# gavrissh/training-operator

Hardware: AMD Instinct MI355X
Metric: job×node fit evals/sec + gang placements/sec, 1M-node inventory, 1/2/4/8 GPUs (higher is better)
Workload: dtype int64

## Files before the change

training-operator_amd/csrc/pe_engine.cpp:

```cpp
#include <hip/hip_runtime.h>
#include <rccl/rccl.h>

#include <immintrin.h>
#include <pthread.h>
#include <sched.h>

#include <algorithm>
#include <deque>
#include <condition_variable>
#include <atomic>
#include <chrono>
#include <exception>
#include <functional>
#include <thread>
#include <cstdio>
#include <cstdlib>
#include <cstring>
#include <memory>
#include <mutex>
#include <new>
#include <numeric>
#include <string>
#include <unordered_map>
#include <vector>
// ... 353 lines not shown
  DevBuf<uint64_t> dm_table;
  HostBuf<uint64_t> dm_hslots;
  HostBuf<uint32_t> dm_hnodes;
  HostBuf<pe::DomPick> dm_hpicks;
  DevBuf<pe::DomPick> dm_picks;
  DevBuf<pe::DomSel> dm_sel;
  HostBuf<pe::DomSel> dm_hsel;
  std::vector<pe::DomPick> dm_upicks;
  std::vector<int32_t> dm_ptab, dm_pof;
  DevBuf<ReqRec> g_groups;
  DevBuf<uint64_t> g_cand, g_bound;
  DevBuf<int32_t> g_cnt;
  DevBuf<uint8_t> g_out, g_gath;
  DevBuf<int64_t> g_upd;
  DevBuf<uint64_t> g_kn;
  DevBuf<uint32_t> g_lo;
  HostBuf<ReqRec> h_groups, h_groups2;
  HostBuf<ReqRec> h_groupsx[2];
  HostBuf<uint8_t> h_outx[2];
  HostBuf<int64_t> h_updx[2];
  uint32_t walk_gen = 0;
  int pin_cpu = -2;
  HostBuf<uint8_t> h_out, h_out2, h_own;
  HostBuf<uint8_t> h_merged;
  HostBuf<uint8_t> h_xg[4];
  std::vector<const uint64_t*> x_lists;
  std::vector<int32_t> x_ns, x_hd;
  HostBuf<int64_t> h_upd;
  bool walk = true;
  int64_t resort_nodes = 20480;
  int64_t w_est = 0;
  struct WalkSet {
    DevBuf<uint64_t> sk, rmin;
    DevBuf<int64_t> sr, rmax;
    DevBuf<uint32_t> sl, pos, ror, inovl, ovidx, ovlab;
    DevBuf<int64_t> ovres;
    DevBuf<uint64_t> ovkn;
    DevBuf<int32_t> ovl, ovln;
    void release() {
      sk.release(); rmin.release(); sr.release(); rmax.release(); sl.release(); pos.release(); ror.release();
      inovl.release(); ovidx.release(); ovlab.release(); ovres.release(); ovkn.release(); ovl.release(); ovln.release();
    }
  } ws[2];
  int w_cur = 0;
  bool w_pending = false;
  int64_t w_pend_est = 0;
  int64_t w_pend_windows = 0;
  hipStream_t w_s2 = nullptr;
  hipEvent_t w_ev_snap = nullptr, w_ev_done = nullptr;
  DevBuf<uint64_t> w_kin;
  DevBuf<uint32_t> w_slow;
  DevBuf<uint8_t> w_temp;
  DevBuf<uint32_t> w_flush;
  DevBuf<unsigned long long> w_stat;
  DevBuf<uint64_t> g_xstatus;
  pe_stats stats{};

  ~pe_ctx() {
    (void)hipSetDevice(device);
    if (comm_abort.joinable()) comm_abort.join();
    if (stream) (void)hipStreamSynchronize(stream);
    res0.release(); res.release(); labels.release(); island.release(); n_upd.release();
    fit_jobs.release(); fit_jobs32.release(); res32.release(); mask.release();
    code_vals.release(); code_needs.release(); code_jobs.release(); code_x.release(); counts.release(); h_counts.release();
    planes.release(); plane_jobs.release();
    lds_spec_d.release(); lds_vals.release(); lds_codes.release(); lds_ranks.release(); lds_aux.release(); lds_slots.release(); lds_rows.release();
    a_stage.release(); a_outh.release(); a_segoff.release(); a_flag.release(); a_ctr.release();
    for (hipEvent_t e : a_ev) (void)hipEventDestroy(e);
    if (a_h2d) (void)hipStreamSynchronize(a_h2d);
    for (hipEvent_t e : a_ev_h2d) (void)hipEventDestroy(e);
    if (a_h2d) (void)hipStreamDestroy(a_h2d);
    a_dstage.release();
    a_jgo.release(); a_mm.release(); a_rep.release(); a_gco.release(); a_mem.release();
    a_req.release(); a_out.release(); a_fl.release(); a_pres.release(); a_ovf.release();
    aw_stage.release(); aw_outh.release(); aw_dev.release();
    cp_hshapes.release(); cp_hout.release(); cp_shapes.release(); cp_part.release(); cp_out.release();
    dm_table.release(); dm_hslots.release(); dm_hnodes.release(); dm_hpicks.release();
    dm_picks.release(); dm_sel.release(); dm_hsel.release();
    for (hipEvent_t e : cp_ev)
      if (e) (void)hipEventDestroy(e);
    g_groups.release(); g_cand.release(); g_bound.release(); g_cnt.release(); g_out.release(); g_gath.release();
    g_upd.release(); g_kn.release(); g_lo.release(); h_groups.release(); h_groups2.release(); h_out.release(); h_out2.release(); h_own.release(); h_merged.release(); h_upd.release();
    for (auto& x : h_xg) x.release();
    for (int i = 0; i < 2; ++i) {
      h_groupsx[i].release();
      h_outx[i].release();
      h_updx[i].release();
    }
    if (w_s2) (void)hipStreamSynchronize(w_s2);
    for (auto& x : ws) x.release();
    w_kin.release(); w_slow.release(); w_temp.release(); w_stat.release(); w_flush.release(); g_xstatus.release();
    if (w_ev_snap) (void)hipEventDestroy(w_ev_snap);
    if (w_ev_done) (void)hipEventDestroy(w_ev_done);
    if (w_s2) (void)hipStreamDestroy(w_s2);
    if (comm) (void)ncclCommDestroy(comm);
    if (stream) (void)hipStreamDestroy(stream);
  }
};

namespace {

void rccl_abort(pe_ctx* ctx) {
  if (!ctx->comm) return;
  ncclComm_t c = ctx->comm;
  ctx->comm = nullptr;
  ctx->comm_aborted = true;
  const int dev = ctx->device;
  ctx->comm_abort = std::thread([c, dev] {
    (void)hipSetDevice(dev);
    (void)ncclCommAbort(c);
  });
}

template <class F>
int guarded(pe_ctx* ctx, F&& body) {
  if (!ctx) return PE_EINVAL;
  std::lock_guard<std::mutex> lk(ctx->mu);
  ctx->err.clear();
  try {
    hipchk(hipSetDevice(ctx->device), "hipSetDevice");
    return body();
  } catch (const PeError& e) {
    ctx->err = e.msg;
    return e.code;
  } catch (const std::bad_alloc&) {
    ctx->err = "host allocation failed";
    return PE_ENOMEM;
  } catch (const pe::CollectiveTimeout& e) {
    ctx->err = e.what();
    rccl_abort(ctx);
    return PE_ERCCL;
  } catch (const pe::ExchangeError& e) {
    ctx->err = e.what();
    return PE_ERCCL;
  } catch (const std::runtime_error& e) {
    ctx->err = e.what();
    return PE_EHIP;
  } catch (...) {
    ctx->err = "unexpected C++ exception";
    return PE_EINVAL;
  }
}

void need_ptr(const void* p, const char* name) {
// ... 2388 lines not shown
      std::vector<double>& d; std::vector<double>& e; std::vector<double>& f;
      ~TraceOut() {
        if (!on || a.empty()) return;
        auto pr = [](const char* n, std::vector<double>& v) {
          if (v.empty()) return;
          std::sort(v.begin(), v.end());
          double sum = 0;
          for (double x : v) sum += x;
          std::fprintf(stderr, "%s n %zu sum %.2f ms mean %.1f us p10 %.1f p50 %.1f p90 %.1f max %.1f\n", n, v.size(),
                       sum / 1e3, sum / v.size(), v[v.size() / 10], v[v.size() / 2], v[v.size() * 9 / 10], v.back());
        };
        pr("wait   ", a);
        pr("resolve", b);
        pr("post   ", c);
        pr("xspin  ", d);
        pr("xmerge ", e);
        pr("xblock ", f);
        auto sib = [](int cpu) {
          char path[128], buf[64] = {0};
          std::snprintf(path, sizeof path, "/sys/devices/system/cpu/cpu%d/topology/thread_siblings_list", cpu);
          FILE* f = std::fopen(path, "r");
          if (f) {
            if (!std::fgets(buf, sizeof buf, f)) buf[0] = 0;
            std::fclose(f);
          }
          buf[std::strcspn(buf, "\n")] = 0;
          return std::string(buf);
        };
        const int mc = sched_getcpu();
        std::fprintf(stderr, "cpus: main %d (siblings %s) helper %d (siblings %s)\n", mc, sib(mc).c_str(), helper_cpu,
                     helper_cpu >= 0 ? sib(helper_cpu).c_str() : "-");
      }
    } trace_out{helper_cpu, trace, tr_wait, tr_res, tr_post, tr_xspin, tr_xmerge, tr_xblock};
    int64_t dump_left = std::getenv("PE_DUMP_MAX_WINDOWS") ? std::atoll(std::getenv("PE_DUMP_MAX_WINDOWS")) : INT64_MAX;
    const size_t gb = pe::cand_group_bytes(K);
    const int Wmax = ctx->window_groups;
    const int Wpad = (int)round_up(Wmax, pe::SC_GT);
    const int nwaves = (int)std::max<int64_t>(1, (ctx->Ns + pe::SC_SPAN - 1) / pe::SC_SPAN);
    hipchk(ctx->g_groups.ensure(Wpad), "alloc groups");
    hipchk(ctx->h_groups.ensure(Wpad, kZeroCopy), "alloc pinned groups");
    hipchk(ctx->g_cand.ensure((size_t)Wpad * nwaves * 64), "alloc cand");
    hipchk(ctx->g_cnt.ensure((size_t)Wpad * nwaves), "alloc cnt");
    hipchk(ctx->g_bound.ensure((size_t)Wpad * nwaves), "alloc bound");
    hipchk(ctx->g_out.ensure((size_t)Wmax * gb), "alloc out");
    hipchk(ctx->h_out.ensure((size_t)Wmax * gb * ctx->world, kZeroCopy), "alloc pinned out");
    if (ctx->pipeline) hipchk(ctx->h_out2.ensure((size_t)Wmax * gb * ctx->world, kZeroCopy), "alloc pinned out");
    if (ctx->world > 1 || ctx->comm) {
      hipchk(ctx->g_gath.ensure((size_t)Wmax * gb * ctx->world), "alloc gather");
      hipchk(ctx->h_own.ensure((size_t)Wmax * gb, kZeroCopy), "alloc pinned own");
    }
    const bool wev = walk && std::getenv("PE_WALK_EVENTS") != nullptr;
    const bool wflush = walk && std::getenv("PE_WALK_FLUSH") != nullptr;
    if (wflush) hipchk(ctx->w_flush.ensure((size_t)512 << 20), "alloc flush buffer");
    std::vector<std::pair<hipEvent_t, hipEvent_t>> walk_events;
    struct EventsFree {
      std::vector<std::pair<hipEvent_t, hipEvent_t>>& v;
      ~EventsFree() {
        for (auto& p : v) {
          (void)hipEventDestroy(p.first);
          (void)hipEventDestroy(p.second);
        }
      }
    } events_free{walk_events};
    int64_t walk_launch_groups = 0;
    std::vector<pe::GroupCands> cands;
    hipStream_t s = ctx->stream;
    const bool use_exchange = ctx->exchange && !(ctx->world == 1 && !ctx->comm);
    const bool pipelined = ctx->pipeline;
    int cb = 0;
    std::unique_ptr<SpinWorker> worker;
    struct Pin {
      cpu_set_t old_set, l3;
      bool on = false;
      Pin(int rank, int world, int& picked) {
        if (std::getenv("PE_NO_PIN") || pthread_getaffinity_np(pthread_self(), sizeof(old_set), &old_set) != 0)
          return;
        if (world > 1 && picked == -2) picked = pe::l3_pick(old_set, rank);
        const int cpu = world > 1 ? picked : sched_getcpu();
        if (!pe::l3_cpus(cpu, &l3)) return;
        CPU_AND(&l3, &l3, &old_set);
        on = CPU_COUNT(&l3) >= 3 && pthread_setaffinity_np(pthread_self(), sizeof(l3), &l3) == 0;
      }
      ~Pin() {
        if (on) (void)pthread_setaffinity_np(pthread_self(), sizeof(old_set), &old_set);
      }
    } pin(ctx->rank, ctx->world, ctx->pin_cpu);
    if (pipelined) {
      worker.reset(new SpinWorker(ctx->device));
      if (pin.on) worker->pin(pin.l3);
    }
    if (pin.on) R.pin_helper(pin.l3);
    auto outbuf = [&](int b) { return b == 0 ? ctx->h_out.p : b == 1 ? ctx->h_out2.p : ctx->h_outx[b - 2].p; };
    auto outbufdev = [&](int b) { return b == 0 ? ctx->h_out.dev : b == 1 ? ctx->h_out2.dev : ctx->h_outx[b - 2].dev; };
    const bool direct_out = ctx->world == 1 && !ctx->comm;
    const bool dev_merge = !direct_out && (int64_t)ctx->world * K <= pe::MG_CAP &&
                           ctx->world <= pe::MG_THREADS / 64 && !std::getenv("PE_HOST_MERGE");
    const bool ranked = (std::getenv("PE_MERGE_RANKED") || (ctx->world <= 2 && !std::getenv("PE_MERGE_SORT"))) &&
                        ctx->world <= pe::RM_MAX_WORLD && pe::merge_ranked_lds(ctx->world, K) <= pe::RM_MAX_LDS;
    auto* const merge_fn = ranked ? &pe::launch_merge_ranked : &pe::launch_merge_shards;
    const bool signalled = pipelined && !std::getenv("PE_NO_GROUP_SIGNAL") && (direct_out ? walk : dev_merge);
    bool zc = false;
    pe_host_exchange* const hx = pe::hx_is(ctx->exchange) ? static_cast<pe_host_exchange*>(ctx->exchange_user) : nullptr;
    if (hx && use_exchange && pipelined && signalled && ctx->walk && !std::getenv("PE_NO_ZC_EXCHANGE")) {
      if (ctx->zc_hx != hx) {
        const uint8_t ok = ctx->world <= pe::HX_ZC_MAX_WORLD && pe::hx_zc_register(hx) &&
                                   (size_t)Wmax * gb <= pe::hx_slot_bytes(hx) ? 1 : 0;
// ... 295 lines not shown
        ctx->stats.xchg_merge_ms += std::chrono::duration<double, std::milli>(std::chrono::steady_clock::now() - tm).count();
      } else if (dev_merge) {
        hipchk(merge_fn(s, ctx->h_xg[b].dev, ctx->world, Wg, K, outbufdev(b), gen, 0, nullptr, true),
               "launch merge_shards");
      }
    };
    auto enqueue_window = [&](const std::vector<int32_t>& groups, int b, uint32_t gen_in = 0, bool defer_x = false,
                              const pe::HxWindow* hw_in = nullptr) {
      const int Wg = (int)groups.size();
      const int Wgp = (int)round_up(Wg, pe::SC_GT);
      const int Kw = rccl_grow ? k_win : K;
      auto& hg = hgroups(b);
      for (int w = 0; w < Wgp; ++w) {
        const int g = groups[std::min(w, Wg - 1)];
        fill_req(hg.p[w], R.scan_req(g), group_need[g]);
      }
      const bool own_direct = walk && use_exchange && pipelined && !zc;
      pe::HxWindow hw;
      if (zc) {
        hw = hw_in ? *hw_in : pe::hx_zc_next(hx);
        if (zc_host && !pe::hx_zc_wait_reuse(hx, hw))
          throw pe::ExchangeError("host exchange: a rank never finished reading a window (peer stalled or failed)");
      }
      uint8_t* const dst = zc           ? hw.dev + (size_t)ctx->rank * hw.slot
                           : direct_out ? outbufdev(b)
                           : own_direct ? ctx->h_own.dev
                                        : ctx->g_out.p;
      uint32_t gen = 0;
      if (gen_in) {
        gen = gen_in;
      } else if (signalled || own_direct) {
        if (++ctx->walk_gen == 0) ++ctx->walk_gen;
        gen = ctx->walk_gen;
      }
      buf_gen[b] = gen;
      buf_k[b] = Kw;
      if (walk) {
        if (ctx->w_pending && (ctx->w_est > ctx->resort_nodes + kResortLate ||
                               (ctx->w_pend_windows++ >= switch_delay && hipEventQuery(ctx->w_ev_done) == hipSuccess)))
          walk_switch(ctx);
        if (!ctx->w_pending) {
          if (async_resort && ctx->w_est > ctx->resort_nodes - kResortEarly) walk_resort_async(ctx);
          else if (ctx->w_est > ctx->resort_nodes) walk_resort(ctx);
        }
        std::pair<hipEvent_t, hipEvent_t> evp{nullptr, nullptr};
        if (wflush) hipchk(hipMemsetD32Async((hipDeviceptr_t)ctx->w_flush.p, ctx->walk_gen, (size_t)128 << 20, s), "flush");
        if (wev) {
          hipchk(hipEventCreate(&evp.first), "event");
          hipchk(hipEventCreate(&evp.second), "event");
          walk_events.push_back(evp);
          hipchk(hipEventRecord(evp.first, s), "event record");
        }
        hipchk(pe::launch_walk(s, hg.dev, Wg, k_win, walk_index(ctx), ctx->res.p, ctx->stride, ctx->labels.p, ctx->Ns,
                               (uint64_t)ctx->begin, dst, zc ? hw.gen : direct_out || own_direct ? gen : 0u, Kw),
               "launch walk");
        if (wev) hipchk(hipEventRecord(evp.second, s), "event record");
        walk_launch_groups += Wg;
      } else if (ctx->Ns > 0) {
        hipchk(hipMemcpyAsync(ctx->g_groups.p, hg.p, Wgp * sizeof(ReqRec), hipMemcpyHostToDevice, s), "H2D window");
        hipchk(pe::launch_scan(s, ctx->res.p, ctx->stride, ctx->labels.p, ctx->g_kn.p, ctx->g_lo.p, ctx->Ns,
                               (uint64_t)ctx->begin, ctx->g_groups.p, Wg, ctx->g_cand.p, ctx->g_cnt.p, ctx->g_bound.p,
                               nwaves),
               "launch scan");
        hipchk(pe::launch_merge(s, ctx->g_cand.p, ctx->g_cnt.p, ctx->g_bound.p, nwaves, K, dst, Wg),
               "launch merge");
      } else if (zc) {
        hipchk(pe::launch_empty_groups(s, Wg, Kw, dst, hw.gen), "launch empty groups");
      } else {
        const size_t gbw = pe::cand_group_bytes(Kw);
        std::vector<uint8_t> empty((size_t)Wg * gbw, 0);
        for (int w = 0; w < Wg; ++w) {
          pe::CandHdr h{0, 0, pe::NO_KEY};
          std::memcpy(empty.data() + (size_t)w * gbw, &h, sizeof(h));
        }
        if (direct_out) {
          std::memcpy(outbuf(b), empty.data(), empty.size());
        } else {
          hipchk(hipMemcpyAsync(dst, empty.data(), empty.size(), hipMemcpyHostToDevice, s), "H2D empty");
          hipchk(hipStreamSynchronize(s), "sync empty");
        }
      }
      const size_t bytes = (size_t)Wg * pe::cand_group_bytes(Kw);
      if (direct_out) {
      } else if (zc_host) {
        ctx->stats.xchg_zc_windows += 1;
        if (!defer_x) exchange_window(b, Wg, gen, false, nullptr, &hw);
      } else if (zc) {
        ctx->stats.xchg_zc_windows += 1;
        hipchk(pe::launch_xwait(s, hw.dev, ctx->world, Wg, K, (int64_t)hw.slot, hw.gen, zc_ticks, ctx->g_xstatus.p),
               "launch exchange wait");
        hipchk(merge_fn(s, hw.dev, ctx->world, Wg, K, outbufdev(b), gen, (int64_t)hw.slot,
                                       ctx->g_xstatus.p, true),
               "launch merge_shards");
      } else if (use_exchange) {
        if (!pipelined)
          hipchk(hipMemcpyAsync(ctx->h_own.p, ctx->g_out.p, bytes, hipMemcpyDeviceToHost, s), "D2H cands");
        else if (!defer_x)
          exchange_window(b, Wg, gen, own_direct, nullptr);
      } else {
        if (stall_window >= 0 && ctx->stats.windows == stall_window && stall_ticks > 0)
          hipchk(pe::launch_stall(s, stall_ticks), "launch stall (test knob)");
        ncclchk(ncclAllGather(ctx->g_out.p, ctx->g_gath.p, bytes, ncclUint8, ctx->comm, s), "ncclAllGather");
        if (dev_merge)
          hipchk(merge_fn(s, ctx->g_gath.p, ctx->world, Wg, Kw, outbufdev(b), gen, 0, nullptr, false),
                 "launch merge_shards");
        else
          hipchk(hipMemcpyAsync(outbuf(b), ctx->g_gath.p, bytes * ctx->world, hipMemcpyDeviceToHost, s),
// ... 325 lines not shown
```

training-operator_amd/csrc/pe_kernels.h:

```cpp
#pragma once
#include <hip/hip_runtime.h>
#include <stdint.h>

namespace pe {

constexpr int D = 4;
constexpr uint64_t SCORE_MAX = (1ull << 40) - 1;
constexpr uint64_t NO_KEY = ~0ull;
constexpr int64_t NEVER = INT64_MIN;

struct alignas(64) ReqRec {
  int64_t q[D];
  uint32_t need;
  uint32_t pad_[7];
};
static_assert(sizeof(ReqRec) == 64, "ReqRec must be 64 B");

struct alignas(32) ReqRec32 {
  int32_t q[D];
  uint32_t need;
  uint32_t pad_[3];
};
static_assert(sizeof(ReqRec32) == 32, "ReqRec32 must be 32 B");

// ... 173 lines not shown
hipError_t launch_scan(hipStream_t s, const int64_t* res, int64_t stride, const uint32_t* labels, const uint64_t* kn,
                       const uint32_t* lo, int64_t Ns, uint64_t id_base, const ReqRec* groups, int Wg, uint64_t* cand,
                       int32_t* cnt, uint64_t* bound, int nwaves);

hipError_t launch_merge(hipStream_t s, const uint64_t* cand, const int32_t* cnt, const uint64_t* bound,
                        int nwaves, int K, uint8_t* out, int Wg);

constexpr int WK_ROUND = 1024;
constexpr int WK_MAXR = 16384;
constexpr uint64_t WK_INVALID = ~0ull;
#ifndef WK_MULTI
#define WK_MULTI 2
#endif
#ifndef WK_MULTI_AFTER
#define WK_MULTI_AFTER 1
#endif
struct WalkIndex {
  uint64_t* sk;
  int64_t* sr;
  uint32_t* sl;
  uint32_t* pos;
  uint64_t* rmin;
  int64_t* rmax;
  uint32_t* ror;
  int32_t* ovl;
  int32_t* ovl_n;
  uint32_t* in_ovl;
  uint32_t* ovl_idx;
  int64_t* ovl_res;
  uint32_t* ovl_lab;
  uint64_t* ovl_kn;
  unsigned long long* stat;
  int64_t sstride, nr;
};
hipError_t launch_walk_prep(hipStream_t s, const int64_t* res, int64_t stride, int64_t Ns, const uint64_t* kn,
                            const uint32_t* labels, uint64_t* kin, const WalkIndex& w, uint32_t* slow = nullptr);
hipError_t launch_walk_switch(hipStream_t s, const int64_t* res, int64_t stride, const uint32_t* labels, int64_t Ns,
                              const uint32_t* slow, const WalkIndex& nx);
hipError_t sort_keys_u64(void* temp, size_t* temp_bytes, const uint64_t* in, uint64_t* out, int64_t n, hipStream_t s);
hipError_t launch_walk_build(hipStream_t s, const int64_t* res, int64_t stride, const uint32_t* labels, int64_t Ns,
                             uint64_t id_base, const WalkIndex& w);
hipError_t launch_merge_shards(hipStream_t s, const uint8_t* gath, int world, int Wg, int K, uint8_t* out, uint32_t gen,
                               int64_t rank_stride = 0, const uint64_t* xstatus = nullptr, bool sys_scope = true);
constexpr int XW_THREADS = 256;
hipError_t launch_xwait(hipStream_t s, const uint8_t* gath, int world, int Wg, int K, int64_t rank_stride,
                        uint32_t in_gen, int64_t timeout_ticks, uint64_t* xstatus);
constexpr int RM_THREADS = 256, RM_MAX_WORLD = 16;
constexpr size_t RM_MAX_LDS = 64 * 1024;
size_t merge_ranked_lds(int world, int K);
hipError_t launch_merge_ranked(hipStream_t s, const uint8_t* gath, int world, int Wg, int K, uint8_t* out, uint32_t gen,
                               int64_t rank_stride = 0, const uint64_t* xstatus = nullptr, bool sys_scope = true);
hipError_t launch_empty_groups(hipStream_t s, int Wg, int K, uint8_t* out, uint32_t gen);
hipError_t launch_stall(hipStream_t s, int64_t ticks);
hipError_t launch_walk(hipStream_t s, const ReqRec* groups, int Wg, int K, const WalkIndex& w, const int64_t* res,
                       int64_t stride, const uint32_t* labels, int64_t Ns, uint64_t id_base, uint8_t* out,
                       uint32_t gen = 0, int K_stride = 0);

hipError_t launch_apply(hipStream_t s, int64_t* res, int64_t stride, const int64_t* upd, int64_t n, uint64_t id_base,
                        uint64_t* kn, uint32_t* lo, const uint32_t* labels, const WalkIndex* w,
                        const WalkIndex* nx = nullptr);

struct NodeUpd {
  int64_t local;
  int64_t res[D];
  uint32_t labels;
  int32_t island;
};
static_assert(sizeof(NodeUpd) == 48, "NodeUpd must be 48 B");
hipError_t launch_scatter_nodes(hipStream_t s, int64_t* res, int64_t* res0, int64_t stride, uint32_t* labels,
                                int32_t* island, const NodeUpd* upd, int64_t n);

constexpr int CP_THREADS = 256;
constexpr int CP_NPT = 4;
constexpr int CP_SPAN = CP_THREADS * CP_NPT;
constexpr int CP_TS = 64;
constexpr uint64_t CP_CAP_MAX = 2147483647;
__host__ __device__ inline int64_t cap_node_blocks(int64_t Ns) { return (Ns + CP_SPAN - 1) / CP_SPAN; }
struct alignas(32) CapShape {
  int64_t q[D];
  uint64_t m[D];
  uint32_t sh[D];
  uint32_t need;
  uint32_t pad_[3];
};
static_assert(sizeof(CapShape) == 96, "CapShape must be 96 B");
struct CapAcc {
  uint64_t slots;
  uint32_t max_node;
  uint32_t nodes;
};
static_assert(sizeof(CapAcc) == 16, "CapAcc must be 16 B");
hipError_t launch_gang_capacity(hipStream_t s, const int64_t* res, int64_t stride, const uint32_t* labels, int64_t Ns,
                                const CapShape* shapes, int64_t S, CapAcc* partials, CapAcc* out);

constexpr int DM_MAX_DOMAINS = 65536;
struct DomPick {
  uint32_t shape;
  int32_t count;
};
struct DomSel {
  uint64_t slots;
  int32_t domain;
  uint32_t feasible;
};
static_assert(sizeof(DomPick) == 8 && sizeof(DomSel) == 16, "DomPick / DomSel layout");
hipError_t launch_gang_capacity_domains(hipStream_t s, const int64_t* res, int64_t stride, const uint32_t* labels,
                                        const int32_t* island, int64_t Ns, const CapShape* shapes, int64_t S,
                                        int n_domains, uint64_t* dom_slots, uint32_t* dom_nodes);
hipError_t launch_domain_select(hipStream_t s, const uint64_t* dom_slots, int64_t s0, int64_t S, int n_domains,
// ... 4 lines not shown
```

training-operator_amd/csrc/pe_kernels.hip:

```cpp
#include <type_traits>

#include "pe_kernels.h"
#include "pe_wave.h"

namespace pe {

__device__ __forceinline__ uint64_t umin64(uint64_t a, uint64_t b) { return a < b ? a : b; }

__device__ __forceinline__ uint64_t wave_min_u64(uint64_t v) {
#pragma unroll
  for (int off = 32; off >= 1; off >>= 1) v = umin64(v, __shfl_xor(v, off, 64));
  return v;
}


__device__ __forceinline__ bool add_ovf(int64_t a, int64_t b, int64_t* r) { return __builtin_add_overflow(a, b, r); }
__device__ __forceinline__ bool mul_ovf(int64_t a, int64_t b, int64_t* r) { return __builtin_mul_overflow(a, b, r); }

template <int ND>
struct AggJob {
  int64_t acc[ND];
  uint32_t pres, members;
  int32_t pod_cnt;
  bool ovf;
// ... 2107 lines not shown
#pragma unroll
  for (int d = 0; d < D; ++d)
    for (int off = 32; off >= 1; off >>= 1) {
      const int64_t o = __shfl_xor(v[d], off, 64);
      v[d] = o > v[d] ? o : v[d];
    }
  for (int off = 32; off >= 1; off >>= 1) lab |= __shfl_xor(lab, off, 64);
  if (lane == 0) {
#pragma unroll
    for (int d = 0; d < D; ++d) mx[d][wave] = v[d];
    orl[wave] = lab;
  }
  __syncthreads();
  if (tid < D) {
    int64_t m = INT64_MIN;
    for (int k = 0; k < WK_ROUND / 64; ++k) m = mx[tid][k] > m ? mx[tid][k] : m;
    w.rmax[tid * w.nr + r] = m;
  } else if (tid == D) {
    uint32_t o = 0;
    for (int k = 0; k < WK_ROUND / 64; ++k) o |= orl[k];
    w.ror[r] = o;
    w.rmin[r] = w.sk[r * WK_ROUND];
  }
}

hipError_t launch_walk_build(hipStream_t s, const int64_t* res, int64_t stride, const uint32_t* labels, int64_t Ns,
                             uint64_t id_base, const WalkIndex& w) {
  if (Ns <= 0) return hipSuccess;
  hipLaunchKernelGGL(walk_build_kernel, dim3((unsigned)w.nr), dim3(WK_ROUND), 0, s, res, stride, labels, Ns, id_base,
                     w);
  return hipGetLastError();
}

__device__ __forceinline__ void step_append(TopkShared& s, int T0, int* cnt, uint64_t k, bool take) {
  const uint64_t bal = __ballot(take);
  if (bal == 0) return;
  const int rank = __builtin_amdgcn_mbcnt_hi((uint32_t)(bal >> 32), __builtin_amdgcn_mbcnt_lo((uint32_t)bal, 0));
  int base = 0;
  if (take && rank == 0) base = atomicAdd(cnt, __popcll(bal));
  base = T0 + __shfl(base, __ffsll((unsigned long long)bal) - 1, 64);
  if (take && base + rank < MG_CAP) s.keys[base + rank] = k;
}

#ifdef PE_WALK_PROF
__device__ unsigned long long walk_prof[32];
#define WPT(i) unsigned long long wpt##i = wall_clock64()
#else
#define WPT(i)
#endif

__global__ __launch_bounds__(WK_ROUND) void walk_kernel(const ReqRec* __restrict__ groups, int K, int Kst, WalkIndex w,
                                                        const int64_t* __restrict__ res, int64_t stride,
                                                        const uint32_t* __restrict__ labels, int64_t Ns,
                                                        uint64_t id_base, uint8_t* __restrict__ out, uint32_t gen) {
  static_assert(WK_ROUND == MG_THREADS, "the walk uses the merge's block-wide selection");
  __shared__ TopkShared s;
  __shared__ uint32_t cbits[WK_MAXR / 32];
  __shared__ int start_cnt, below[2], wcnt[3];
  const int g = blockIdx.x;
  const int tid = threadIdx.x, lane = tid & 63;
  WPT(0);
  const ReqRec rq = groups[g];
  const int64_t q0 = rq.q[0], q1 = rq.q[1], q2 = rq.q[2], q3 = rq.q[3];
  const uint32_t need = rq.need;
  uint64_t sq = (uint64_t)q0 + ((uint64_t)q1 >> 20) + ((uint64_t)q3 >> 24);
  sq = (uint64_t)q0 > SCORE_MAX || (uint64_t)q2 >= (1ull << 20) || sq >= SCORE_MAX ? SCORE_MAX : sq;
  sq = sq < SCORE_MAX ? sq + ((uint64_t)q2 << 20) : sq;
  const bool walk = sq < SCORE_MAX;
  const uint64_t KQ = walk ? sq << 24 : 0;
  const uint64_t KQ2 = !walk ? 0 : sq + 2 >= (1ull << 40) ? ~0ull : (sq + 2) << 24;
  const int64_t nr = w.nr;
  const int nwords = (int)((nr + 31) / 32);
  for (int i = tid; i < nwords; i += WK_ROUND) cbits[i] = 0u;
  if (tid == 0) {
    s.total = 0;
    start_cnt = 0;
    below[0] = below[1] = 0;
    wcnt[0] = wcnt[1] = wcnt[2] = 0;
  }
  __syncthreads();
  if (walk) {
    int cnt = 0;
    for (int64_t r0 = 0; r0 < nr; r0 += WK_ROUND) {
      const int64_t r = r0 + tid;
      bool can = false;
      if (r < nr) {
        cnt += w.rmin[r] < KQ;
        can = q0 <= w.rmax[r] && q1 <= w.rmax[nr + r] && q2 <= w.rmax[2 * nr + r] && q3 <= w.rmax[3 * nr + r] &&
              (w.ror[r] & need) == need;
      }
#ifdef PE_PREPASS_ATOMIC
      if (can) atomicOr(&cbits[r >> 5], 1u << (r & 31));
#else
      const uint64_t bal = __ballot(can);
      const int64_t wr = r0 + (tid & ~63);
      if (lane == 0 && wr < nr) {
        cbits[wr >> 5] = (uint32_t)bal;
        if (wr + 32 < nr) cbits[(wr >> 5) + 1] = (uint32_t)(bal >> 32);
      }
#endif
    }
    for (int off = 32; off >= 1; off >>= 1) cnt += __shfl_xor(cnt, off, 64);
    if (lane == 0 && cnt) atomicAdd(&start_cnt, cnt);
  }
  __syncthreads();
  WPT(1);
  bool done = !walk;
  int rounds = 0;
  int64_t r = walk ? (start_cnt > 0 ? start_cnt - 1 : 0) : nr;
  auto next_round = [&](int64_t from) -> int64_t {
    int64_t wi = from >> 5;
    if (wi >= nwords) return nr;
    uint32_t bits = cbits[wi] & (~0u << (from & 31));
    while (bits == 0) {
      if (++wi >= nwords) return nr;
      bits = cbits[wi];
    }
    return wi * 32 + __ffs(bits) - 1;
  };
  if (!done) r = next_round(r);
  uint64_t xstop = NO_KEY;
  int tests = 0;
  int lo_idx = 0, cnt_certain = 0;
  constexpr int PEND = 4;
  int pend_n = 0;
  int pend_end[PEND];
  uint64_t pend_b[PEND];
  auto pend_push = [&](int end, uint64_t b) {
    if (pend_n == PEND) {
#pragma unroll
      for (int i = 0; i + 1 < PEND; ++i) {
        pend_end[i] = pend_end[i + 1];
        pend_b[i] = pend_b[i + 1];
      }
      --pend_n;
    }
#pragma unroll
    for (int i = 0; i < PEND; ++i)
      if (i == pend_n) {
        pend_end[i] = end;
        pend_b[i] = b;
      }
    ++pend_n;
  };
  int Tcur = 0;
  int step = 0;
  auto compact = [&]() {
    const int T2 = Tcur < MG_CAP ? Tcur : MG_CAP;
    const uint64_t* sk = topk_sort(s, T2, K);
    const int m = T2 < K + 1 ? T2 : K + 1;
    uint64_t v = tid < m ? sk[tid] : 0;
    __syncthreads();
    if (tid < m) s.keys[tid] = v;
    __syncthreads();
    Tcur = m;
    return m;
  };
  auto step_begin = [&]() -> int* {
    if (tid == 0) wcnt[(step + 1) % 3] = 0;
    return &wcnt[step % 3];
  };
  auto step_end = [&]() {
// ... 71 lines not shown
    }
    int64_t rr[WK_MULTI];
    int nstep = 1;
    rr[0] = r;
    if (rounds >= WK_MULTI_AFTER)
      for (; nstep < WK_MULTI; ++nstep) {
        const int64_t nx = next_round(rr[nstep - 1] + 1);
        if (nx >= nr) break;
        rr[nstep] = nx;
      }
    const int64_t r_next = next_round(rr[nstep - 1] + 1);
    const uint64_t rm_next = r_next < nr ? w.rmin[r_next] : 0;
    uint64_t k[WK_MULTI];
#pragma unroll
    for (int u = 0; u < WK_MULTI; ++u) {
      k[u] = NO_KEY;
      const int64_t i = rr[u < nstep ? u : 0] * WK_ROUND + tid;
      if (u < nstep && i < Ns) {
#ifdef PE_WALK_COND_LOAD
        const uint64_t Kn = w.sk[i];
        if (Kn != WK_INVALID)
          k[u] = node_key(w.sr[i], w.sr[w.sstride + i], w.sr[2 * w.sstride + i], w.sr[3 * w.sstride + i], w.sl[i], q0,
                          q1, q2, q3, need, Kn & 0xFFFFFFull);
#else
        const uint64_t Kn = w.sk[i];
        const int64_t s0 = w.sr[i], s1 = w.sr[w.sstride + i], s2 = w.sr[2 * w.sstride + i], s3 = w.sr[3 * w.sstride + i];
        const uint32_t sl = w.sl[i];
        const uint64_t kk = node_key(s0, s1, s2, s3, sl, q0, q1, q2, q3, need, Kn & 0xFFFFFFull);
        k[u] = Kn != WK_INVALID ? kk : NO_KEY;
#endif
      }
    }
    int* const cnt = step_begin();
#pragma unroll
    for (int u = 0; u < WK_MULTI; ++u)
      if (u < nstep) step_append(s, Tcur, cnt, k[u], k[u] != NO_KEY);
    __syncthreads();
    step_end();
    pend_push(Tcur, r_next < nr ? (rm_next > KQ ? rm_next - KQ : 0) : NO_KEY);
    if (Tcur > MG_CAP - WK_MULTI * WK_ROUND) {
      const int m = compact();
      lo_idx = cnt_certain = pend_n = 0;
      pend_push(m, m > 0 ? s.keys[m - 1] : 0);
    }
    r = r_next;
    rm_r = rm_next;
    rounds += nstep;
  }
  WPT(2);
#ifndef WK_OV
#define WK_OV 8
#endif
  constexpr int OV = WK_OV;
  const int no = *w.ovl_n;
  const uint64_t klim = xstop > NO_KEY - KQ2 ? NO_KEY : xstop + KQ2;
  for (int i0 = 0; i0 < no; i0 += OV * WK_ROUND) {
    uint64_t kn[OV];
#pragma unroll
    for (int u = 0; u < OV; ++u) {
      const int i = i0 + u * WK_ROUND + tid;
      kn[u] = i < no ? w.ovl_kn[i] : 0;
    }
    uint64_t k[OV];
#pragma unroll
    for (int u = 0; u < OV; ++u) {
      const int i = i0 + u * WK_ROUND + tid;
      k[u] = NO_KEY;
      if (i < no && (kn[u] == KEY_SLOW || (kn[u] >= KQ && kn[u] < klim)))
        k[u] = node_key(w.ovl_res[i], w.ovl_res[w.sstride + i], w.ovl_res[2 * w.sstride + i],
                        w.ovl_res[3 * w.sstride + i], w.ovl_lab[i], q0, q1, q2, q3, need, id_base + (uint64_t)w.ovl[i]);
    }
    if (Tcur > MG_CAP - OV * WK_ROUND) compact();
    int* const cnt = step_begin();
#pragma unroll
    for (int u = 0; u < OV; ++u) step_append(s, Tcur, cnt, k[u], k[u] < xstop);
    __syncthreads();
    step_end();
  }
  __syncthreads();
  WPT(3);
  const int T = Tcur < MG_CAP ? Tcur : MG_CAP;
  const uint64_t* sk = topk_sort(s, T, K, xstop);
  WPT(4);
  write_group(sk, T < K ? T : K, 0, T > K ? sk[K] : NO_KEY, Kst, g, out, gen);
  if (tid == 0 && w.stat) {
    atomicAdd(&w.stat[0], (unsigned long long)rounds);
    atomicAdd(&w.stat[1], (unsigned long long)no);
  }
#ifdef PE_WALK_PROF
  __syncthreads();
  WPT(5);
  if (tid == 0) {
    atomicAdd(&walk_prof[0], wpt1 - wpt0);
    atomicAdd(&walk_prof[1], wpt2 - wpt1);
    atomicAdd(&walk_prof[2], wpt3 - wpt2);
    atomicAdd(&walk_prof[3], wpt4 - wpt3);
    atomicAdd(&walk_prof[4], wpt5 - wpt4);
    atomicAdd(&walk_prof[5], 1ull);
    atomicAdd(&walk_prof[6], (unsigned long long)no);
    atomicAdd(&walk_prof[7], (unsigned long long)rounds);
    atomicAdd(&walk_prof[8], (unsigned long long)T);
    atomicMax(&walk_prof[9], wpt5 - wpt0);
    atomicMax(&walk_prof[10], wpt2 - wpt1);
    atomicMax(&walk_prof[11], wpt3 - wpt2);
    atomicMax(&walk_prof[12], wpt4 - wpt3);
    atomicMax(&walk_prof[13], (unsigned long long)rounds);
    atomicMax(&walk_prof[14], (unsigned long long)T);
    atomicMax(&walk_prof[15], wpt1 - wpt0);
    if (wpt5 - wpt0 > 3500) {
      atomicAdd(&walk_prof[16], 1ull);
      atomicAdd(&walk_prof[17], wpt1 - wpt0);
      atomicAdd(&walk_prof[18], wpt2 - wpt1);
      atomicAdd(&walk_prof[19], wpt3 - wpt2);
      atomicAdd(&walk_prof[20], wpt4 - wpt3);
      atomicAdd(&walk_prof[21], wpt5 - wpt4);
      atomicAdd(&walk_prof[22], (unsigned long long)rounds);
      atomicAdd(&walk_prof[23], (unsigned long long)T);
      atomicAdd(&walk_prof[24], (unsigned long long)no);
      atomicAdd(&walk_prof[25], (unsigned long long)tests);
    }
  }
#endif
}

hipError_t launch_walk(hipStream_t s, const ReqRec* groups, int Wg, int K, const WalkIndex& w, const int64_t* res,
                       int64_t stride, const uint32_t* labels, int64_t Ns, uint64_t id_base, uint8_t* out,
                       uint32_t gen, int K_stride) {
  if (Wg <= 0) return hipSuccess;
  const int Kst = K_stride > 0 ? K_stride : K;
  if (w.nr > WK_MAXR || K + 1 > WK_ROUND || K > Kst) return hipErrorInvalidValue;
  hipLaunchKernelGGL(walk_kernel, dim3((unsigned)Wg), dim3(WK_ROUND), 0, s, groups, K, Kst, w, res, stride, labels, Ns,
                     id_base, out, gen);
#ifdef PE_WALK_PROF
  static int launches = 0;
  if (++launches % 500 == 0) {
    unsigned long long p[32];
    (void)hipStreamSynchronize(s);
    (void)hipMemcpyFromSymbol(p, HIP_SYMBOL(walk_prof), sizeof(p));
    const double n = (double)p[5], us = 100.0;
    fprintf(stderr, "walk prof over %.0f blocks (us/block): setup+prepass %.2f walk %.2f overlay %.2f sort %.2f write %.2f"
                    " | overlay %.0f rounds %.2f T %.0f\n", n, p[0] / n / us, p[1] / n / us, p[2] / n / us,
            p[3] / n / us, p[4] / n / us, p[6] / n, p[7] / n, p[8] / n);
    fprintf(stderr, "walk prof max: block %.2f us setup %.2f walk %.2f overlay %.2f sort %.2f | rounds %llu T %llu\n",
            p[9] / us, p[15] / us, p[10] / us, p[11] / us, p[12] / us, p[13], p[14]);
    const double ns = (double)(p[16] ? p[16] : 1);
    fprintf(stderr, "walk prof slow blocks (> 35 us): %.0f (%.2f%%): setup %.2f walk %.2f overlay %.2f sort %.2f write %.2f"
                    " us | rounds %.2f T %.0f overlay %.0f tests %.2f\n", (double)p[16], 100.0 * p[16] / n, p[17] / ns / us,
            p[18] / ns / us, p[19] / ns / us, p[20] / ns / us, p[21] / ns / us, p[22] / ns, p[23] / ns, p[24] / ns, p[25] / ns);
    unsigned long long t[8];
    (void)hipMemcpyFromSymbol(t, HIP_SYMBOL(topk_prof), sizeof(t));
    const double c = (double)t[0];
    fprintf(stderr, "topk_sort: %.0f calls, T %.0f, C %.0f, bitonic %.0f, hist+select %.2f us, rank %.2f us per call\n",
            c, t[1] / c, t[3] / c, (double)t[2], t[4] / c / us, t[5] / c / us);
  }
#endif
  return hipGetLastError();
}


__global__ __launch_bounds__(256) void apply_kernel(int64_t* __restrict__ res, int64_t stride,
                                                    const int64_t* __restrict__ upd, int64_t n, uint64_t id_base,
                                                    uint64_t* __restrict__ kn, uint32_t* __restrict__ lo,
                                                    const uint32_t* __restrict__ labels, WalkIndex w, int walk,
                                                    WalkIndex nx, int pend) {
  const int64_t i = (int64_t)blockIdx.x * blockDim.x + threadIdx.x;
  if (i >= n) return;
  const int64_t* u = upd + i * (D + 1);
  const int64_t node = u[0];
#pragma unroll
  for (int d = 0; d < D; ++d) res[d * stride + node] = u[1 + d];
  uint64_t K;
  uint32_t l1, l3;
  node_prep(u[1], u[2], u[3], u[4], id_base + (uint64_t)node, K, l1, l3);
  if (kn) {
    kn[node] = K;
    lo[node] = l1;
    lo[stride + node] = l3;
  }
  if (walk) {
    const uint32_t p = w.pos[node];
    if (p != ~0u) {
      w.sk[p] = WK_INVALID;
      w.pos[node] = ~0u;
    }
    const int64_t r[D] = {u[1], u[2], u[3], u[4]};
    if (atomicExch(&w.in_ovl[node], 1u) == 0u) {
      overlay_add(w, node, r, labels[node], K);
    } else {
      const uint32_t i = w.ovl_idx[node];
#pragma unroll
      for (int d = 0; d < D; ++d) w.ovl_res[d * w.sstride + i] = r[d];
      w.ovl_kn[i] = K;
    }
    if (pend) {
      if (atomicExch(&nx.in_ovl[node], 1u) == 0u) {
        overlay_add(nx, node, r, labels[node], K);
      } else {
        const uint32_t i = nx.ovl_idx[node];
#pragma unroll
        for (int d = 0; d < D; ++d) nx.ovl_res[d * nx.sstride + i] = r[d];
        nx.ovl_kn[i] = K;
// ... 42 lines not shown
```

Before: 46390 billion.

## Split walk kernel into separate round-walk and overlay blocks merged via scratch

Each walk group is now handled by two blocks, one doing the index round walk and one scanning the overlay list. Each block writes its local top-K+1 keys to global scratch, and whichever finishes second merges both lists with a binary-search merge in shared memory and writes the group output. The goal is to cut per-group latency by running the two phases in parallel across more blocks. In exchange it doubles the block count, adds global-memory handoff and atomics, and relies on the scratch counter parity being correct across launches. This path is on by default when walking and can be disabled with PE_WALK_SPLIT=0.

```diff
diff --git a/training-operator_amd/csrc/pe_engine.cpp b/training-operator_amd/csrc/pe_engine.cpp
--- a/training-operator_amd/csrc/pe_engine.cpp
+++ b/training-operator_amd/csrc/pe_engine.cpp
@@ -429,6 +429,7 @@
   DevBuf<uint32_t> w_slow;
   DevBuf<uint8_t> w_temp;
   DevBuf<uint32_t> w_flush;
+  DevBuf<uint64_t> w_split;
   DevBuf<unsigned long long> w_stat;
   DevBuf<uint64_t> g_xstatus;
   pe_stats stats{};
@@ -466,7 +467,7 @@
     }
     if (w_s2) (void)hipStreamSynchronize(w_s2);
     for (auto& x : ws) x.release();
-    w_kin.release(); w_slow.release(); w_temp.release(); w_stat.release(); w_flush.release(); g_xstatus.release();
+    w_kin.release(); w_slow.release(); w_temp.release(); w_stat.release(); w_flush.release(); w_split.release(); g_xstatus.release();
     if (w_ev_snap) (void)hipEventDestroy(w_ev_snap);
     if (w_ev_done) (void)hipEventDestroy(w_ev_done);
     if (w_s2) (void)hipStreamDestroy(w_s2);
@@ -2961,6 +2962,11 @@
     const bool wev = walk && std::getenv("PE_WALK_EVENTS") != nullptr;
     const bool wflush = walk && std::getenv("PE_WALK_FLUSH") != nullptr;
     if (wflush) hipchk(ctx->w_flush.ensure((size_t)512 << 20), "alloc flush buffer");
+    const bool wsplit = walk && !(std::getenv("PE_WALK_SPLIT") && std::atoi(std::getenv("PE_WALK_SPLIT")) == 0);
+    if (wsplit && ctx->w_split.n < pe::walk_split_words(Wmax)) {
+      hipchk(ctx->w_split.ensure(pe::walk_split_words(Wmax)), "alloc walk split scratch");
+      hipchk(hipMemsetAsync(ctx->w_split.p, 0, ctx->w_split.n * sizeof(uint64_t), ctx->stream), "memset walk split scratch");
+    }
     std::vector<std::pair<hipEvent_t, hipEvent_t>> walk_events;
     struct EventsFree {
       std::vector<std::pair<hipEvent_t, hipEvent_t>>& v;
@@ -3362,7 +3368,8 @@
           hipchk(hipEventRecord(evp.first, s), "event record");
         }
         hipchk(pe::launch_walk(s, hg.dev, Wg, k_win, walk_index(ctx), ctx->res.p, ctx->stride, ctx->labels.p, ctx->Ns,
-                               (uint64_t)ctx->begin, dst, zc ? hw.gen : direct_out || own_direct ? gen : 0u, Kw),
+                               (uint64_t)ctx->begin, dst, zc ? hw.gen : direct_out || own_direct ? gen : 0u, Kw,
+                               wsplit ? ctx->w_split.p : nullptr),
                "launch walk");
         if (wev) hipchk(hipEventRecord(evp.second, s), "event record");
         walk_launch_groups += Wg;
diff --git a/training-operator_amd/csrc/pe_kernels.h b/training-operator_amd/csrc/pe_kernels.h
--- a/training-operator_amd/csrc/pe_kernels.h
+++ b/training-operator_amd/csrc/pe_kernels.h
@@ -249,9 +249,12 @@
                                int64_t rank_stride = 0, const uint64_t* xstatus = nullptr, bool sys_scope = true);
 hipError_t launch_empty_groups(hipStream_t s, int Wg, int K, uint8_t* out, uint32_t gen);
 hipError_t launch_stall(hipStream_t s, int64_t ticks);
+constexpr int WS_HDR = 16;
+constexpr int WS_GROUP = WS_HDR + 2 * WK_ROUND;
+inline size_t walk_split_words(int Wg) { return (size_t)(Wg > 0 ? Wg : 0) * WS_GROUP; }
 hipError_t launch_walk(hipStream_t s, const ReqRec* groups, int Wg, int K, const WalkIndex& w, const int64_t* res,
                        int64_t stride, const uint32_t* labels, int64_t Ns, uint64_t id_base, uint8_t* out,
-                       uint32_t gen = 0, int K_stride = 0);
+                       uint32_t gen = 0, int K_stride = 0, uint64_t* split = nullptr);
 
 hipError_t launch_apply(hipStream_t s, int64_t* res, int64_t stride, const int64_t* upd, int64_t n, uint64_t id_base,
                         uint64_t* kn, uint32_t* lo, const uint32_t* labels, const WalkIndex* w,
diff --git a/training-operator_amd/csrc/pe_kernels.hip b/training-operator_amd/csrc/pe_kernels.hip
--- a/training-operator_amd/csrc/pe_kernels.hip
+++ b/training-operator_amd/csrc/pe_kernels.hip
@@ -2183,12 +2183,20 @@
 __global__ __launch_bounds__(WK_ROUND) void walk_kernel(const ReqRec* __restrict__ groups, int K, int Kst, WalkIndex w,
                                                         const int64_t* __restrict__ res, int64_t stride,
                                                         const uint32_t* __restrict__ labels, int64_t Ns,
-                                                        uint64_t id_base, uint8_t* __restrict__ out, uint32_t gen) {
+                                                        uint64_t id_base, uint8_t* __restrict__ out, uint32_t gen,
+                                                        int Wg, uint64_t* __restrict__ split) {
   static_assert(WK_ROUND == MG_THREADS, "the walk uses the merge's block-wide selection");
   __shared__ TopkShared s;
   __shared__ uint32_t cbits[WK_MAXR / 32];
   __shared__ int start_cnt, below[2], wcnt[3];
-  const int g = blockIdx.x;
+  int g = blockIdx.x, role = -1;
+  if (split) {
+    g = (int)(blockIdx.x >> 4) * 8 + (int)(blockIdx.x & 7);
+    role = (int)(blockIdx.x >> 3) & 1;
+    if (g >= Wg) return;
+  }
+  const bool do_rounds = role != 1, do_ovl = role != 0;
+  uint64_t* const sp = split ? split + (size_t)g * WS_GROUP : nullptr;
   const int tid = threadIdx.x, lane = tid & 63;
   WPT(0);
   const ReqRec rq = groups[g];
@@ -2202,7 +2210,8 @@
   const uint64_t KQ2 = !walk ? 0 : sq + 2 >= (1ull << 40) ? ~0ull : (sq + 2) << 24;
   const int64_t nr = w.nr;
   const int nwords = (int)((nr + 31) / 32);
-  for (int i = tid; i < nwords; i += WK_ROUND) cbits[i] = 0u;
+  if (do_rounds)
+    for (int i = tid; i < nwords; i += WK_ROUND) cbits[i] = 0u;
   if (tid == 0) {
     s.total = 0;
     start_cnt = 0;
@@ -2210,7 +2219,7 @@
     wcnt[0] = wcnt[1] = wcnt[2] = 0;
   }
   __syncthreads();
-  if (walk) {
+  if (walk && do_rounds) {
     int cnt = 0;
     for (int64_t r0 = 0; r0 < nr; r0 += WK_ROUND) {
       const int64_t r = r0 + tid;
@@ -2236,9 +2245,9 @@
   }
   __syncthreads();
   WPT(1);
-  bool done = !walk;
+  bool done = !walk || !do_rounds;
   int rounds = 0;
-  int64_t r = walk ? (start_cnt > 0 ? start_cnt - 1 : 0) : nr;
+  int64_t r = !done ? (start_cnt > 0 ? start_cnt - 1 : 0) : nr;
   auto next_round = [&](int64_t from) -> int64_t {
     int64_t wi = from >> 5;
     if (wi >= nwords) return nr;
@@ -2416,7 +2425,7 @@
 #define WK_OV 8
 #endif
   constexpr int OV = WK_OV;
-  const int no = *w.ovl_n;
+  const int no = do_ovl ? *w.ovl_n : 0;
   const uint64_t klim = xstop > NO_KEY - KQ2 ? NO_KEY : xstop + KQ2;
   for (int i0 = 0; i0 < no; i0 += OV * WK_ROUND) {
     uint64_t kn[OV];
@@ -2446,10 +2455,52 @@
   const int T = Tcur < MG_CAP ? Tcur : MG_CAP;
   const uint64_t* sk = topk_sort(s, T, K, xstop);
   WPT(4);
-  write_group(sk, T < K ? T : K, 0, T > K ? sk[K] : NO_KEY, Kst, g, out, gen);
+  if (role < 0) {
+    write_group(sk, T < K ? T : K, 0, T > K ? sk[K] : NO_KEY, Kst, g, out, gen);
+  } else {
+    __shared__ int second;
+    const int m = T < K + 1 ? T : K + 1;
+    const uint64_t own = tid < m ? sk[tid] : NO_KEY;
+    if (tid < m) __hip_atomic_store(&sp[WS_HDR + role * WK_ROUND + tid], own, __ATOMIC_RELAXED, __HIP_MEMORY_SCOPE_AGENT);
+    if (tid == 0) __hip_atomic_store(&sp[1 + role], (uint64_t)m, __ATOMIC_RELAXED, __HIP_MEMORY_SCOPE_AGENT);
+    asm volatile("s_waitcnt vmcnt(0)" ::: "memory");
+    __syncthreads();
+    if (tid == 0)
+      second = (int)(__hip_atomic_fetch_add(&sp[0], 1ull, __ATOMIC_RELAXED, __HIP_MEMORY_SCOPE_AGENT) & 1ull);
+    __syncthreads();
+    if (second) {
+      const uint64_t* pl = sp + WS_HDR + (1 - role) * WK_ROUND;
+      int mp = (int)__hip_atomic_load(&sp[1 + (1 - role)], __ATOMIC_RELAXED, __HIP_MEMORY_SCOPE_AGENT);
+      mp = mp < 0 ? 0 : mp > K + 1 ? K + 1 : mp;
+      const uint64_t pk = tid < mp ? __hip_atomic_load(&pl[tid], __ATOMIC_RELAXED, __HIP_MEMORY_SCOPE_AGENT) : NO_KEY;
+      uint64_t* const pls = s.keys + WK_ROUND;
+      uint64_t* const mg = s.keys + 2 * WK_ROUND;
+      if (tid < mp) pls[tid] = pk;
+      __syncthreads();
+      if (tid < m) {
+        int lo = 0, hi = mp;
+        while (lo < hi) {
+          const int mid = (lo + hi) >> 1;
+          if (pls[mid] < own) lo = mid + 1; else hi = mid;
+        }
+        if (tid + lo <= K) mg[tid + lo] = own;
+      }
+      if (tid < mp) {
+        int lo = 0, hi = m;
+        while (lo < hi) {
+          const int mid = (lo + hi) >> 1;
+          if (sk[mid] <= pk) lo = mid + 1; else hi = mid;
+        }
+        if (tid + lo <= K) mg[tid + lo] = pk;
+      }
+      __syncthreads();
+      const int M = m + mp;
+      write_group(mg, M < K ? M : K, 0, M > K ? mg[K] : NO_KEY, Kst, g, out, gen);
+    }
+  }
   if (tid == 0 && w.stat) {
-    atomicAdd(&w.stat[0], (unsigned long long)rounds);
-    atomicAdd(&w.stat[1], (unsigned long long)no);
+    if (do_rounds) atomicAdd(&w.stat[0], (unsigned long long)rounds);
+    if (do_ovl) atomicAdd(&w.stat[1], (unsigned long long)no);
   }
 #ifdef PE_WALK_PROF
   __syncthreads();
@@ -2483,18 +2534,27 @@
       atomicAdd(&walk_prof[24], (unsigned long long)no);
       atomicAdd(&walk_prof[25], (unsigned long long)tests);
     }
+    if (role == 1) {
+      atomicAdd(&walk_prof[26], 1ull);
+      atomicAdd(&walk_prof[27], wpt5 - wpt0);
+      atomicAdd(&walk_prof[28], wpt3 - wpt2);
+      atomicAdd(&walk_prof[29], wpt4 - wpt3);
+      atomicAdd(&walk_prof[30], wpt5 - wpt4);
+      atomicAdd(&walk_prof[31], (unsigned long long)T);
+    }
   }
 #endif
 }
 
 hipError_t launch_walk(hipStream_t s, const ReqRec* groups, int Wg, int K, const WalkIndex& w, const int64_t* res,
                        int64_t stride, const uint32_t* labels, int64_t Ns, uint64_t id_base, uint8_t* out,
-                       uint32_t gen, int K_stride) {
+                       uint32_t gen, int K_stride, uint64_t* split) {
   if (Wg <= 0) return hipSuccess;
   const int Kst = K_stride > 0 ? K_stride : K;
   if (w.nr > WK_MAXR || K + 1 > WK_ROUND || K > Kst) return hipErrorInvalidValue;
-  hipLaunchKernelGGL(walk_kernel, dim3((unsigned)Wg), dim3(WK_ROUND), 0, s, groups, K, Kst, w, res, stride, labels, Ns,
-                     id_base, out, gen);
+  const unsigned blocks = split ? (unsigned)((Wg + 7) / 8) * 16u : (unsigned)Wg;
+  hipLaunchKernelGGL(walk_kernel, dim3(blocks), dim3(WK_ROUND), 0, s, groups, K, Kst, w, res, stride, labels, Ns,
+                     id_base, out, gen, Wg, split);
 #ifdef PE_WALK_PROF
   static int launches = 0;
   if (++launches % 500 == 0) {
@@ -2511,6 +2571,11 @@
     fprintf(stderr, "walk prof slow blocks (> 35 us): %.0f (%.2f%%): setup %.2f walk %.2f overlay %.2f sort %.2f write %.2f"
                     " us | rounds %.2f T %.0f overlay %.0f tests %.2f\n", (double)p[16], 100.0 * p[16] / n, p[17] / ns / us,
             p[18] / ns / us, p[19] / ns / us, p[20] / ns / us, p[21] / ns / us, p[22] / ns, p[23] / ns, p[24] / ns, p[25] / ns);
+    if (p[26]) {
+      const double no = (double)p[26];
+      fprintf(stderr, "walk prof overlay blocks: %.0f: block %.2f overlay %.2f sort %.2f handoff+write %.2f us | T %.0f\n", no,
+              p[27] / no / us, p[28] / no / us, p[29] / no / us, p[30] / no / us, p[31] / no);
+    }
     unsigned long long t[8];
     (void)hipMemcpyFromSymbol(t, HIP_SYMBOL(topk_prof), sizeof(t));
     const double c = (double)t[0];
```

Measured after the change: 46380 billion. No clear change (-0.0%).
